# wuxiaolang/Cube_SLAM_wu

Measured on AMD Instinct MI355X. Metric: frames/sec detect_cuboid, higher is better.
Workload: dtype f64

## Files before the change

cube_slam_wu_amd/csrc/detect_kernels.hip:

```cpp
#include <hip/hip_runtime.h>
#include "cs_hip_util.h"

#include <cstdio>
#include <cstdlib>
#include <cstring>

#include "../../include/cubeslam_hip.h"
#include "detect_types.h"

namespace cs {

__device__ __forceinline__ int wave_uniform_i32(int x) { return __builtin_amdgcn_readfirstlane(x); }
__device__ __forceinline__ long long wave_uniform_i64(long long x) {
  const unsigned lo = (unsigned)__builtin_amdgcn_readfirstlane((int)(unsigned)(x & 0xffffffffll)), hi = (unsigned)__builtin_amdgcn_readfirstlane((int)(x >> 32));
  return (long long)(((unsigned long long)hi << 32) | lo);
}
template <typename T>
__device__ __forceinline__ int find_job_wave(const T* __restrict__ prefix, int n, T elem) {
  const T first = sizeof(T) == 8 ? (T)wave_uniform_i64((long long)elem) : (T)wave_uniform_i32((int)elem);
  int lo = 0, hi = n;
  while (hi - lo > 1) {
    const int mid = (lo + hi) >> 1;
    if (prefix[mid] <= first) lo = mid; else hi = mid;
  }
  while (lo + 1 < n && prefix[lo + 1] <= elem) lo++;
  return lo;
}

__device__ __forceinline__ long long xcd_virtual_block() {
  long long nb = gridDim.x, b = blockIdx.x;
  return (b & 7) * (nb >> 3) + (b >> 3);
}

__device__ __attribute__((noinline)) double vp_exact_raw(double dy, double dx) { return cs_atan2(dy, dx); }

__device__ __forceinline__ double vp_exact_unwrapped(const double* __restrict__ mx, const double* __restrict__ my, int i, int ib, double vpxk, double vpyk) {
  const double raw = vp_exact_raw(my[i] - vpyk, mx[i] - vpxk);
  if (i == ib) return raw;
  const double base = vp_exact_raw(my[ib] - vpyk, mx[ib] - vpxk);
  if ((raw - base) < -CS_PI) return raw + 2 * CS_PI;
  if ((raw - base) > CS_PI) return raw - 2 * CS_PI;
  return raw;
}
__device__ __attribute__((noinline)) float vp_rare_unwrapped_f(const double* mx, const double* my, int i, int ib, double vpxk, double vpyk) {
  return (float)vp_exact_unwrapped(mx, my, i, ib, vpxk, vpyk);
}
__device__ __attribute__((noinline)) bool vp_rare_greater(const double* mx, const double* my, int i, int i_ref, int ib, double vpxk, double vpyk) {
  return vp_exact_unwrapped(mx, my, i, ib, vpxk, vpyk) > vp_exact_unwrapped(mx, my, i_ref, ib, vpxk, vpyk);
}
__device__ __attribute__((noinline)) bool vp_rare_less(const double* mx, const double* my, int i, int i_ref, int ib, double vpxk, double vpyk) {
  return vp_exact_unwrapped(mx, my, i, ib, vpxk, vpyk) < vp_exact_unwrapped(mx, my, i_ref, ib, vpxk, vpyk);
}
struct VpExactInlier { float at; int inl; };
__device__ __attribute__((noinline)) VpExactInlier vp_rare_inlier(double dyd, double dxd, double lai, double thre) {
  const double raw = cs_atan2(dyd, dxd);
  const double nrm = normalize_to_pi(raw);
  double d = dabs(lai - nrm);
  d = dmin(d, CS_PI - d);
  return VpExactInlier{(float)raw, d < thre ? 1 : 0};
}

struct VpRun {
  bool have;
  int ib, i_hi, i_lo;
  float base_f, hi_f, lo_f;
  double hx, hy, lx, ly;
};

__device__ __forceinline__ float atan2_float(float fy, float fx, bool* usable) {
  const float PI_F = 3.14159274f, HPI_F = 1.57079637f;
  const float ay = fabsf(fy), ax = fabsf(fx);
  const float hi = fmaxf(ax, ay), lo = fminf(ax, ay);
  const float q = lo * __builtin_amdgcn_rcpf(hi), q2 = q * q;
  float at = -0.01172120f;
  at = __builtin_fmaf(at, q2, 0.05265332f);
  at = __builtin_fmaf(at, q2, -0.11643287f);
  at = __builtin_fmaf(at, q2, 0.19354346f);
  at = __builtin_fmaf(at, q2, -0.33262347f);
  at = __builtin_fmaf(at, q2, 0.99997726f);
  at = at * q;
  if (ay > ax) at = HPI_F - at;
  if (fx < 0.0f) at = PI_F - at;
  if (fy < 0.0f) at = -at;
  *usable = hi > 0.0f && hi < 3.0e38f;
  return at;
}

__device__ __forceinline__ void vp_step(const double* __restrict__ mx, const double* __restrict__ my, int i, double mxi, double myi, double lai,
                                        double vpxk, double vpyk, double thre, float thre_f, VpRun& R) {
  const float PI_F = 3.14159274f, HPI_F = 1.57079637f, M_IN = 1.0e-5f, M_ORD = 2.0e-5f;
  const double dyd = myi - vpyk, dxd = mxi - vpxk;
  bool usable;
  float at = atan2_float((float)dyd, (float)dxd, &usable);
  float nr = at;
  if (at > HPI_F) nr = at - PI_F; else if (at < -HPI_F) nr = at + PI_F;
  float df = fabsf((float)lai - nr);
  df = fminf(df, PI_F - df);
  bool inl = usable && df < thre_f - M_IN;
  if (!(inl || (usable && df > thre_f + M_IN))) { const VpExactInlier x = vp_rare_inlier(dyd, dxd, lai, thre); inl = x.inl != 0; at = x.at; }
  if (inl) {
    if (!R.have) {
      R.have = true; R.ib = i; R.i_hi = i; R.i_lo = i; R.base_f = at; R.hi_f = at; R.lo_f = at; R.hx = dxd; R.hy = dyd; R.lx = dxd; R.ly = dyd;
    } else {
      const float d = at - R.base_f;
      float sh = d < -PI_F ? at + 2.0f * PI_F : d > PI_F ? at - 2.0f * PI_F : at;
      if (fabsf(fabsf(d) - PI_F) < M_ORD) sh = vp_rare_unwrapped_f(mx, my, i, R.ib, vpxk, vpyk);
      if (sh > R.hi_f + M_ORD) { R.hi_f = sh; R.i_hi = i; R.hx = dxd; R.hy = dyd; }
      else if (sh > R.hi_f - M_ORD) {
        const double c = R.hx * dyd - R.hy * dxd, lim = 1.0e-12 * ((dabs(dxd) + dabs(dyd)) * (dabs(R.hx) + dabs(R.hy)));
        const bool greater = c > lim ? true : c < -lim ? false : vp_rare_greater(mx, my, i, R.i_hi, R.ib, vpxk, vpyk);
        if (greater) { R.hi_f = sh; R.i_hi = i; R.hx = dxd; R.hy = dyd; }
      }
      if (sh < R.lo_f - M_ORD) { R.lo_f = sh; R.i_lo = i; R.lx = dxd; R.ly = dyd; }
      else if (sh < R.lo_f + M_ORD) {
        const double c = R.lx * dyd - R.ly * dxd, lim = 1.0e-12 * ((dabs(dxd) + dabs(dyd)) * (dabs(R.lx) + dabs(R.ly)));
        const bool less = c < -lim ? true : c > lim ? false : vp_rare_less(mx, my, i, R.i_lo, R.ib, vpxk, vpyk);
        if (less) { R.lo_f = sh; R.i_lo = i; R.lx = dxd; R.ly = dyd; }
      }
    }
  }
}

struct VpChunk {
  double2 xy[64];
  double ang[64];
  float2 dir[64];
};

template <int K, bool UNIFORM>
__device__ __forceinline__ void vp_support_multi(const double* __restrict__ mx, const double* __restrict__ my, const double* __restrict__ la, int m, VpChunk* ch,
                                                 const double* vpx, const double* vpy, const double* thre, const bool* swapped, bool lane_on, double* out) {
  VpRun R[K];
  float thre_f[K], tan_f[K];
#pragma unroll
  for (int k = 0; k < K; k++) {
    R[k] = VpRun{false, 0, 0, 0, 0.f, 0.f, 0.f, 0., 0., 0., 0.}; thre_f[k] = (float)thre[k];
    tan_f[k] = thre_f[k] < 1.5f ? tanf(thre_f[k] + 1.0e-4f) : __builtin_huge_valf();
  }
  if (UNIFORM) {
    const int lane = threadIdx.x & 63;
    for (int c0 = 0; c0 < m; c0 += 64) {
      const int n = min(64, m - c0);
      __builtin_amdgcn_fence(__ATOMIC_ACQ_REL, "wavefront");
      if (lane < n) {
        const double a = la[c0 + lane];
        ch->xy[lane] = make_double2(mx[c0 + lane], my[c0 + lane]);
        ch->ang[lane] = a;
        ch->dir[lane] = make_float2(cosf((float)a), sinf((float)a));
      }
      __builtin_amdgcn_fence(__ATOMIC_ACQ_REL, "wavefront");
      __builtin_amdgcn_wave_barrier();
      unsigned long long mask[K];
#pragma unroll
      for (int k = 0; k < K; k++) mask[k] = 0;
#pragma unroll 4
      for (int u = 0; u < n; u++) {
        const double2 P = ch->xy[u];
        const float2 ud = ch->dir[u];
#pragma unroll
        for (int k = 0; k < K; k++) {
          const float fx = (float)(P.x - vpx[k]), fy = (float)(P.y - vpy[k]);
          const float cr = fabsf(__builtin_fmaf(fx, ud.y, -(fy * ud.x))), dt = fabsf(__builtin_fmaf(fx, ud.x, fy * ud.y));
          const bool out_for_sure = cr > __builtin_fmaf(tan_f[k], dt, 2.0e-6f * (fabsf(fx) + fabsf(fy)));
          mask[k] |= (unsigned long long)(out_for_sure ? 0 : 1) << u;
        }
      }
#pragma unroll
      for (int k = 0; k < K; k++) {
        unsigned long long mk = lane_on ? mask[k] : 0ull;
        while (__any(mk != 0)) {
          if (mk != 0) {
            const int u = __ffsll((long long)mk) - 1;
            mk &= mk - 1;
            const double2 P = ch->xy[u];
            vp_step(mx, my, c0 + u, P.x, P.y, ch->ang[u], vpx[k], vpy[k], thre[k], thre_f[k], R[k]);
          }
        }
      }
    }
  } else {
    const int mm = lane_on ? m : 0;
    for (int i = 0; i < mm; i++) {
      const double X = mx[i], Y = my[i], A = la[i];
#pragma unroll
      for (int k = 0; k < K; k++) vp_step(mx, my, i, X, Y, A, vpx[k], vpy[k], thre[k], thre_f[k], R[k]);
    }
  }
  const double NaN = __builtin_nan("");
#pragma unroll
  for (int k = 0; k < K; k++) {
    const double ang_hi = R[k].have ? la[R[k].i_hi] : NaN, ang_lo = R[k].have ? la[R[k].i_lo] : NaN;
    out[2 * k] = swapped[k] ? ang_lo : ang_hi;
    out[2 * k + 1] = swapped[k] ? ang_hi : ang_lo;
  }
}

enum { VP3_RPCAP = 32 };

template <int MODE, bool UNIFORM>
__device__ __forceinline__ void vp_support_body(const DetectDeviceView& v, const SweepParams& sp, const JobDesc& jd, int j, long long e, bool on, VpChunk* ch) {
  int rp = 0, y = 0;
  if (on) {
    int local = (int)e - jd.vp_off;
    on = local < jd.RP * jd.Y;
    rp = local / jd.Y; y = local - rp * jd.Y;
  }
  double vpx[3] = {0, 0, 0}, vpy[3] = {0, 0, 0};
  if (on) {
    const RpPose* pose = v.rp + jd.rp_off + rp;
    double cy = v.yaw_cos[jd.yaw_off + y], sy = v.yaw_sin[jd.yaw_off + y];
    const double* A = pose->KinvR;
    double d[3][3] = {{cy, sy, 0.0}, {-sy, cy, 0.0}, {0.0, 0.0, 1.0}};
#pragma unroll
    for (int k = 0; k < 3; k++) {
      double h0 = (A[0] * d[k][0] + A[1] * d[k][1]) + A[2] * d[k][2];
      double h1 = (A[3] * d[k][0] + A[4] * d[k][1]) + A[5] * d[k][2];
      double h2 = (A[6] * d[k][0] + A[7] * d[k][1]) + A[8] * d[k][2];
      vpx[k] = h0 / h2;
      vpy[k] = h1 / h2;
    }
    if (MODE == 0) {
      double* vout = v.vp + 6 * e;
      vout[0] = vpx[0]; vout[1] = vpy[0]; vout[2] = vpx[1]; vout[3] = vpy[1]; vout[4] = vpx[2]; vout[5] = vpy[2];
    }
  }
  const double* mx = v.mid_x + jd.line_off;
  const double* my = v.mid_y + jd.line_off;
  const double* la = v.line_angle + jd.line_off;
  double b6[6];
  const double thre[3] = {sp.vp12_thre_rad, sp.vp12_thre_rad, sp.vp3_thre_rad};
  const bool swapped[3] = {false, true, true};
  vp_support_multi<(MODE == 0 ? 3 : 2), UNIFORM>(mx, my, la, jd.m, ch, vpx, vpy, thre, swapped, on, b6);
  if (!on) return;
  if (MODE == 1) { const double* t3 = v.bound3 + 2 * ((size_t)j * VP3_RPCAP + rp); b6[4] = t3[0]; b6[5] = t3[1]; }
  double* bout = v.bound + 6 * e;
#pragma unroll
  for (int q = 0; q < 6; q++) bout[q] = b6[q];
}

template <int MODE>
__global__ __launch_bounds__(256) void vp_support_kernel(DetectDeviceView v, SweepParams sp, int vp_total) {
  long long e = xcd_virtual_block() * blockDim.x + threadIdx.x;
  const bool on = e < vp_total;
  const int j = find_job_wave<int>(v.vp_prefix, v.n_jobs, on ? (int)e : vp_total - 1);
  const int ju = wave_uniform_i32(j);
  __shared__ VpChunk chunk[4];
  if (__all(j == ju)) vp_support_body<MODE, true>(v, sp, v.jobs[ju], ju, e, on, &chunk[threadIdx.x >> 6]);
  else vp_support_body<MODE, false>(v, sp, v.jobs[j], j, e, on, nullptr);
}

__global__ __launch_bounds__(64) void vp3_support_kernel(DetectDeviceView v, SweepParams sp, int rp_stride) {
  const long long e = (long long)blockIdx.x * 64 + threadIdx.x;
  const int j = (int)(e / rp_stride), rp = (int)(e % rp_stride);
  bool on = j < v.n_jobs;
  JobDesc jd{};
  if (on) { jd = v.jobs[j]; on = rp < jd.RP && jd.Y > 0; }
  double vx = 0, vy = 0;
  if (on) {
    const double* A = (v.rp + jd.rp_off + rp)->KinvR;
    double h0 = (A[0] * 0.0 + A[1] * 0.0) + A[2] * 1.0;
    double h1 = (A[3] * 0.0 + A[4] * 0.0) + A[5] * 1.0;
    double h2 = (A[6] * 0.0 + A[7] * 0.0) + A[8] * 1.0;
    vx = h0 / h2; vy = h1 / h2;
  }
  double o2[2];
  const bool swapped3 = true;
  vp_support_multi<1, false>(v.mid_x + jd.line_off, v.mid_y + jd.line_off, v.line_angle + jd.line_off, on ? jd.m : 0, nullptr, &vx, &vy, &sp.vp3_thre_rad, &swapped3, on, o2);
  if (on) { double* t3 = v.bound3 + 2 * ((size_t)j * VP3_RPCAP + rp); t3[0] = o2[0]; t3[1] = o2[1]; }
}

__global__ __launch_bounds__(256) void vp_points_kernel(DetectDeviceView v, int vp_total) {
  long long e = (long long)blockIdx.x * blockDim.x + threadIdx.x;
  int j = find_job_wave<int>(v.vp_prefix, v.n_jobs, e < vp_total ? (int)e : vp_total - 1);
  if (e >= vp_total) return;
  const JobDesc jd = v.jobs[j];
  int local = (int)e - jd.vp_off;
  if (local >= jd.RP * jd.Y) return;
  int rp = local / jd.Y, y = local - rp * jd.Y;
  const RpPose* pose = v.rp + jd.rp_off + rp;
  double cy = v.yaw_cos[jd.yaw_off + y], sy = v.yaw_sin[jd.yaw_off + y];
  const double* A = pose->KinvR;
  double d[3][3] = {{cy, sy, 0.0}, {-sy, cy, 0.0}, {0.0, 0.0, 1.0}};
  double* vout = v.vp + 6 * e;
#pragma unroll
  for (int k = 0; k < 3; k++) {
    double h0 = (A[0] * d[k][0] + A[1] * d[k][1]) + A[2] * d[k][2];
    double h1 = (A[3] * d[k][0] + A[4] * d[k][1]) + A[5] * d[k][2];
    double h2 = (A[6] * d[k][0] + A[7] * d[k][1]) + A[8] * d[k][2];
    vout[2 * k] = h0 / h2;
    vout[2 * k + 1] = h1 / h2;
  }
}

__device__ __forceinline__ int candidate_one(const DetectDeviceView& v, const SweepParams& sp, const JobDesc& jd, long long tid) {
  const unsigned k = (unsigned)(tid - jd.slot_off);
  const unsigned half = (unsigned)jd.RP * (unsigned)jd.Y * (unsigned)jd.T;
  if (k >= 2 * half) { v.flag[tid] = 0; return 0; }
  const int cfg = (k >= half) ? 2 : 1;
  const unsigned rest = (k >= half) ? k - half : k;
  const unsigned ryu = rest / (unsigned)jd.T;
  const int t = (int)(rest - ryu * (unsigned)jd.T);
  const long long slot = jd.slot_off + (long long)rest * 2 + (cfg - 1);
  const bool enabled = (cfg == 1) ? (sp.consider_config_1 != 0) : (sp.consider_config_2 != 0);
  int flag = 0;
  if (enabled) {
    const double* vp = v.vp + 6 * (long long)(jd.vp_off + (int)ryu);
    V2 c[8];
    flag = build_corners(jd.g, v2(vp[0], vp[1]), v2(vp[2], vp[3]), v2(vp[4], vp[5]), (double)v.top_x[jd.top_off + t], cfg, sp.short_sq_bound, c);
  }
  v.flag[slot] = flag;
  return flag;
}

__global__ __launch_bounds__(256) void candidate_kernel(DetectDeviceView v, SweepParams sp, long long slot_total) {
  long long tid = xcd_virtual_block() * blockDim.x + threadIdx.x;
  bool active = tid < slot_total;
  int flag = 0;
  int j = find_job_wave<long long>(v.slot_prefix, v.n_jobs, active ? tid : slot_total - 1);
  const int ju = wave_uniform_i32(j);
  if (__all(j == ju)) {
    if (active) flag = candidate_one(v, sp, v.jobs[ju], tid);
  } else {
    if (active) flag = candidate_one(v, sp, v.jobs[j], tid);
  }
  unsigned long long valid = __ballot(flag != 0);
  if (valid) {
    int lane = threadIdx.x & 63;
    int j0 = __shfl(j, __ffsll((long long)valid) - 1);
    unsigned long long same = __ballot(flag != 0 && j == j0);
    if (same == valid) {
      if (lane == __ffsll((long long)valid) - 1) atomicAdd(&v.job_valid[j0], __popcll(valid));
    } else if (flag != 0) {
      atomicAdd(&v.job_valid[j], 1);
    }
  }
}

enum { COMPACT_PER = 16 };
enum { CC_TRIP = 4096 };
__global__ __launch_bounds__(256) void candidate_compact_kernel(DetectDeviceView v, SweepParams sp) {
  const int j = blockIdx.x;
  if (j >= v.n_jobs) return;
  __shared__ unsigned char s_flag[CC_TRIP];
  __shared__ int wsum[4];
  const JobDesc& jd = v.jobs[j];
  const int tid = threadIdx.x, lane = tid & 63, wid = tid >> 6;
  const int n_vp = jd.RP * jd.Y;
  for (int e = tid; e < n_vp; e += 256) {
    const int rp = e / jd.Y, y = e - rp * jd.Y;
    const RpPose* pose = v.rp + jd.rp_off + rp;
    const double cy = v.yaw_cos[jd.yaw_off + y], sy = v.yaw_sin[jd.yaw_off + y];
    const double* A = pose->KinvR;
    const double d[3][3] = {{cy, sy, 0.0}, {-sy, cy, 0.0}, {0.0, 0.0, 1.0}};
    double* vout = v.vp + 6 * (long long)(jd.vp_off + e);
#pragma unroll
    for (int k = 0; k < 3; k++) {
      const double h0 = (A[0] * d[k][0] + A[1] * d[k][1]) + A[2] * d[k][2];
      const double h1 = (A[3] * d[k][0] + A[4] * d[k][1]) + A[5] * d[k][2];
      const double h2 = (A[6] * d[k][0] + A[7] * d[k][1]) + A[8] * d[k][2];
      vout[2 * k] = h0 / h2;
      vout[2 * k + 1] = h1 / h2;
    }
  }
  __syncthreads();
  const unsigned half = (unsigned)n_vp * (unsigned)jd.T;
  const unsigned Tu = (unsigned)jd.T;
  const bool fast_div = Tu > 1 && (unsigned long long)half * Tu < (1ull << 32);
  const unsigned inv_T = fast_div ? 0xffffffffu / Tu + 1u : 0u;
  const long long base = v.slot_prefix[j];
  long long run = base;
  const unsigned long long below = (1ull << lane) - 1ull;
  const bool en1 = sp.consider_config_1 != 0, en2 = sp.consider_config_2 != 0;
  for (unsigned r0 = 0; r0 < half; r0 += CC_TRIP / 2) {
#pragma unroll 1
    for (int q = 0; q < 16; q++) {
      const int cfg = 1 + (q >> 3);
      const unsigned rl = (unsigned)(q & 7) * 256u + (unsigned)tid, rest = r0 + rl;
      int flag = 0;
      if (rest < half && (cfg == 1 ? en1 : en2)) {
        const unsigned ryu = fast_div ? __umulhi(rest, inv_T) : rest / Tu;
        const int t = (int)(rest - ryu * Tu);
        const double* vp = v.vp + 6 * (long long)(jd.vp_off + (int)ryu);
        V2 c[8];
        flag = build_corners(jd.g, v2(vp[0], vp[1]), v2(vp[2], vp[3]), v2(vp[4], vp[5]), (double)v.top_x[jd.top_off + t], cfg, sp.short_sq_bound, c);
      }
      s_flag[2 * rl + (unsigned)(cfg - 1)] = (unsigned char)flag;
    }
    __syncthreads();
    int f[COMPACT_PER];
    int wcount = 0;
#pragma unroll
    for (int q = 0; q < COMPACT_PER; q++) {
      f[q] = s_flag[wid * (64 * COMPACT_PER) + q * 64 + lane];
      wcount += __popcll(__ballot(f[q] != 0));
    }
    if (lane == 0) wsum[wid] = wcount;
    __syncthreads();
    int woff = 0, total = 0;
#pragma unroll
    for (int w = 0; w < 4; w++) { const int x = wsum[w]; if (w < wid) woff += x; total += x; }
    long long pos0 = run + woff;
    const long long sl0 = base + 2ll * r0 + wid * (64 * COMPACT_PER) + lane;
#pragma unroll
    for (int q = 0; q < COMPACT_PER; q++) {
      const unsigned long long bal = __ballot(f[q] != 0);
      if (f[q] != 0) {
        const long long pos = pos0 + __popcll(bal & below);
        v.c_slot[pos] = sl0 + q * 64;
        v.c_flag[pos] = f[q] | (j << CAND_JOB_SHIFT);
      }
      pos0 += __popcll(bal);
    }
    run += total;
    __syncthreads();
  }
  const int n_valid = (int)(run - base);
  if (tid == 0) { v.job_valid[j] = n_valid; v.job_cbase[j] = base; }
  const int nblk = (n_valid + 255) >> 8;
  if (nblk > 0) {
    __shared__ int s_at;
    if (tid == 0) s_at = atomicAdd(&v.blk_info[0], nblk);
    __syncthreads();
    const int at = s_at, b0 = (int)(base >> 8);
    for (int k = tid; k < nblk; k += 256) {
      const int left = n_valid - 256 * k;
      v.blk_info[2 + 2 * (long long)(at + k)] = b0 + k;
      v.blk_info[3 + 2 * (long long)(at + k)] = left > 256 ? 256 : left;
    }
  }
}

__device__ __forceinline__ int slot_corners(const DetectDeviceView& v, const JobDesc& jd, long long slot, double short_sq_bound, V2 c[8]) {
  const unsigned local = (unsigned)(slot - jd.slot_off);
  const unsigned rest = local >> 1, ryu = rest / (unsigned)jd.T;
  const int t = (int)(rest - ryu * (unsigned)jd.T);
  const double* vp = v.vp + 6 * (long long)(jd.vp_off + (int)ryu);
  return build_corners(jd.g, v2(vp[0], vp[1]), v2(vp[2], vp[3]), v2(vp[4], vp[5]), (double)v.top_x[jd.top_off + t], (int)(local & 1) + 1, short_sq_bound, c);
}
__device__ __forceinline__ void slot_corners16(const DetectDeviceView& v, long long slot, double short_sq_bound, double out16[16]) {
  int lo = 0, hi = v.n_jobs;
  while (hi - lo > 1) { const int mid = (lo + hi) >> 1; if (v.slot_prefix[mid] <= slot) lo = mid; else hi = mid; }
  V2 c[8];
#pragma unroll
  for (int q = 0; q < 8; q++) c[q] = v2(0.0, 0.0);
  slot_corners(v, v.jobs[lo], slot, short_sq_bound, c);
#pragma unroll
  for (int q = 0; q < 8; q++) { out16[q] = c[q].x; out16[8 + q] = c[q].y; }
}

__device__ __forceinline__ int sel(int cfg, int a, int b) { return cfg ? b : a; }

enum { SCORE_JOBS = 4, SCORE_SUB = 128, SCORE_BINS = SCORE_JOBS * SCORE_SUB };
__device__ __forceinline__ unsigned score_udiv(unsigned n, unsigned d, unsigned inv) { return inv ? __umulhi(n, inv) : n / d; }
template <bool CAP>
__global__ __launch_bounds__(256) void score_kernel(DetectDeviceView v, long long slot_total, double short_sq_bound) {
  __shared__ double C16[16][260];
  double (*CXt)[260] = C16, (*CYt)[260] = C16 + 8;
  const bool cap = CAP;
  long long n_valid = cap ? 256ll * v.blk_info[0] : v.job_cbase[v.n_jobs];
  const long long per_xcd = ((n_valid + 255) / 256 + 7) / 8;
  const long long kx = blockIdx.x >> 3;
  if (kx >= per_xcd) return;
  long long base = ((long long)(blockIdx.x & 7) * per_xcd + kx) * blockDim.x;
  if (base >= n_valid) return;
  if (cap) {
    const int* entry = v.blk_info + 2 + 2 * (base >> 8);
    base = 256ll * entry[0];
    n_valid = base + entry[1];
  }
  __shared__ int hist[SCORE_BINS + 1];
  __shared__ int s_src[256], s_job[256], s_flag[256];
  __shared__ long long s_slot[256];
  {
    const int t0 = threadIdx.x;
    for (int b = t0; b <= SCORE_BINS; b += 256) hist[b] = 0;
    __syncthreads();
    const long long i0 = base + t0;
    long long slot0 = 0;
    int j0 = 0;
    int flag0 = 0;
    if (i0 < n_valid) { slot0 = v.c_slot[i0]; flag0 = v.c_flag[i0]; j0 = flag0 >> CAND_JOB_SHIFT; }
    s_slot[t0] = slot0; s_job[t0] = j0; s_flag[t0] = flag0 & CAND_VP_MASK;
    __syncthreads();
    int key = SCORE_BINS;
    if (i0 < n_valid) {
      const int jq = CAP ? __builtin_amdgcn_readfirstlane(s_job[0]) : j0;
      const int T0 = v.jobs[jq].T;
      const unsigned loc = (unsigned)(slot0 - v.jobs[jq].slot_off);
      const int jrel = j0 - s_job[0];
      const unsigned hq = loc >> 1;
      const unsigned qT = CAP ? score_udiv(hq, (unsigned)T0, ((unsigned long long)v.jobs[jq].RP * v.jobs[jq].Y * T0 * T0 < (1ull << 32) && T0 > 1) ? 0xffffffffu / (unsigned)T0 + 1u : 0u) : hq / (unsigned)T0;
      const int sub = (int)(loc & 1) * T0 + (int)(hq - qT * (unsigned)T0);
      key = (jrel < SCORE_JOBS && sub < SCORE_SUB) ? jrel * SCORE_SUB + sub : SCORE_BINS - 1;
    }
    const int rank = atomicAdd(&hist[key], 1);
    __syncthreads();
    if (t0 < 64) {
      constexpr int PER = (SCORE_BINS + 1 + 63) / 64;
      int loc_sum = 0, vals[PER];
#pragma unroll
      for (int q = 0; q < PER; q++) { const int b = t0 * PER + q; vals[q] = b <= SCORE_BINS ? hist[b] : 0; loc_sum += vals[q]; }
      int incl = loc_sum;
#pragma unroll
      for (int o = 1; o < 64; o <<= 1) { const int y = __shfl_up(incl, o); if (t0 >= o) incl += y; }
      int run = incl - loc_sum;
#pragma unroll
      for (int q = 0; q < PER; q++) { const int b = t0 * PER + q; if (b <= SCORE_BINS) hist[b] = run; run += vals[q]; }
    }
    __syncthreads();
    s_src[hist[key] + rank] = t0;
    __syncthreads();
  }
  const int mine = s_src[threadIdx.x];
  const JobDesc& jd = v.jobs[CAP ? __builtin_amdgcn_readfirstlane(s_job[0]) : s_job[mine]];
  const long long i = base + mine;
  if (i >= n_valid) return;
  const long long slot = s_slot[mine];
  const unsigned local = (unsigned)(slot - jd.slot_off);
  const int cfg = (int)(local & 1);
  const unsigned inv_T = (CAP && jd.T > 1 && (unsigned long long)jd.RP * jd.Y * jd.T * jd.T < (1ull << 32)) ? 0xffffffffu / (unsigned)jd.T + 1u : 0u;
  const unsigned inv_Y = (CAP && jd.Y > 1 && (unsigned long long)jd.RP * jd.Y * jd.Y < (1ull << 32)) ? 0xffffffffu / (unsigned)jd.Y + 1u : 0u;
  const int ry = (int)score_udiv(local >> 1, (unsigned)jd.T, inv_T);
  const int rp = (int)score_udiv((unsigned)ry, (unsigned)jd.Y, inv_Y);
  const int tx = threadIdx.x;
  const double ox = (double)jd.g.el, oy = (double)jd.g.et;
  const float* __restrict__ map = v.maps + jd.map_off;
  {
    V2 cb[8];
    const unsigned rest = local >> 1;
    const double* vp = v.vp + 6 * (long long)(jd.vp_off + ry);
    rebuild_accepted_corners(jd.g, v2(vp[0], vp[1]), v2(vp[2], vp[3]), v2(vp[4], vp[5]), (double)v.top_x[jd.top_off + (int)(rest - (unsigned)ry * (unsigned)jd.T)], cfg + 1,
                             s_flag[mine], cb);
#pragma unroll
    for (int q = 0; q < 8; q++) { CXt[q][tx] = cb[q].x; CYt[q][tx] = cb[q].y; }
  }
  double bnd[6];
  {
    const double* bound = v.bound + 6 * (long long)(jd.vp_off + ry);
#pragma unroll
    for (int q = 0; q < 6; q++) bnd[q] = bound[q];
  }
  float sum_dist = 0;
  const unsigned long long EA = cfg ? 0x004213210ull : 0x443213210ull, EB = cfg ? 0x005450321ull : 0x577450321ull;
  const unsigned long long EW = cfg ? 0x004332222ull : 0x222222222ull;
  const int n_edges = cfg ? 7 : 9;
  const int map_w = jd.map_w;
  constexpr int EU = 3;
  const bool wave_has_cfg1 = __any(cfg == 0);
#pragma unroll 1
  for (int e0 = 0; e0 < n_edges; e0 += EU) {
    float dv[EU][11];
#pragma unroll
    for (int u = 0; u < EU; u++) {
      const int e = e0 + u;
      if (u > 0 && e0 == 6 && !wave_has_cfg1) {
#pragma unroll
        for (int s = 0; s < 11; s++) dv[u][s] = 0.0f;
        continue;
      }
      const int a = (int)((EA >> (4 * e)) & 7), b = (int)((EB >> (4 * e)) & 7);
      const double x1 = CXt[a][tx] - ox, y1 = CYt[a][tx] - oy, x2 = CXt[b][tx] - ox, y2 = CYt[b][tx] - oy;
#pragma unroll
      for (int s = 0; s < 11; s++) {
        double sx, sy;
        if (s == 0) { sx = x2; sy = y2; }
        else if (s == 10) { sx = x1; sy = y1; }
        else if (s == 5) { sx = (x1 + x2) * 0.5; sy = (y1 + y2) * 0.5; }
        else { const double w = (double)s / 10.0; sx = w * x1 + (1 - w) * x2; sy = w * y1 + (1 - w) * y2; }
        dv[u][s] = map[(unsigned)(__mul24((int)sy, map_w) + (int)sx)];
      }
    }
#pragma unroll
    for (int u = 0; u < EU; u++) {
      const int e = e0 + u;
      const float wt = 0.5f * (float)(int)((EW >> (4 * e)) & 7);
      const bool on = e < n_edges;
#pragma unroll
      for (int s = 0; s < 11; s++) { const float nx = sum_dist + dv[u][s] * wt; sum_dist = on ? nx : sum_dist; }
    }
  }
  double total = 0;
  const double not_found_penalty = 30.0 / 180.0 * CS_PI * 2;
  const int ID1[3][4] = {{0, 1, 7, 4}, {3, 0, 4, 5}, {3, 7, 1, 5}}, ID2[3][4] = {{0, 1, 2, 3}, {3, 0, 4, 5}, {2, 4, 1, 5}};
#pragma unroll
  for (int k = 0; k < 3; k++) {
    double b0 = bnd[2 * k], b1 = bnd[2 * k + 1];
    bool v0 = !(b0 != b0), v1 = !(b1 != b1);
    if (v0 || v1) {
#pragma unroll
      for (int ee = 0; ee < 2; ee++) {
        int pa = sel(cfg, ID1[k][2 * ee], ID2[k][2 * ee]), pb = sel(cfg, ID1[k][2 * ee + 1], ID2[k][2 * ee + 1]);
        double ang = normalize_to_pi(cs_atan2(CYt[pb][tx] - CYt[pa][tx], CXt[pb][tx] - CXt[pa][tx]));
        double best = 100;
        if (v0) { double t = dabs(ang - b0); t = dmin(t, CS_PI - t); if (t < best) best = t; }
        if (v1) { double t = dabs(ang - b1); t = dmin(t, CS_PI - t); if (t < best) best = t; }
        total = total + best;
      }
    } else {
      total = total + not_found_penalty;
    }
  }
  V2 c[8];
#pragma unroll
  for (int q = 0; q < 8; q++) c[q] = v2(CXt[q][tx], CYt[q][tx]);
  const RpPose* pose = v.rp + jd.rp_off + rp;
  double p3[3], s3[3];
  lift_to_3d(c, pose->R, pose->t, v.invK + 9 * jd.frame, pose->plane, p3, s3);
  int flag = s_flag[mine];
  if (s3[0] < 0 || s3[1] < 0 || s3[2] < 0) flag |= CAND_NEG_SCALE;
  v.c_flag[i] = flag;
  v.c_dist[i] = (double)sum_dist / jd.diag;
  v.c_angle[i] = total;
  v.c_skew[i] = dmax(s3[0], s3[1]) / dmin(s3[0], s3[1]);
}

__global__ __launch_bounds__(1024) void scan_jobs_kernel(const int* job_valid, long long* job_cbase, int n_jobs) {
  __shared__ long long wsum[16];
  __shared__ long long carry_s;
  if (threadIdx.x == 0) carry_s = 0;
  __syncthreads();
  int lane = threadIdx.x & 63, wid = threadIdx.x >> 6;
  for (int base = 0; base < n_jobs; base += 1024) {
    int i = base + threadIdx.x;
    long long x = (i < n_jobs) ? job_valid[i] : 0;
    long long incl = x;
#pragma unroll
    for (int o = 1; o < 64; o <<= 1) {
      long long y = __shfl_up(incl, o);
      if (lane >= o) incl += y;
    }
    if (lane == 63) wsum[wid] = incl;
    __syncthreads();
    long long woff = 0;
    for (int w = 0; w < wid; w++) woff += wsum[w];
    long long carry = carry_s;
    if (i < n_jobs) job_cbase[i] = carry + woff + incl - x;
    __syncthreads();
    if (threadIdx.x == 1023) carry_s = carry + woff + incl;
    __syncthreads();
  }
  if (threadIdx.x == 0) job_cbase[n_jobs] = carry_s;
}

__global__ __launch_bounds__(256) void compact_kernel(DetectDeviceView v) {
  int j = blockIdx.x;
  if (j >= v.n_jobs) return;
  __shared__ int wsum[4];
  const long long s0 = v.slot_prefix[j], s1 = v.slot_prefix[j + 1];
  long long run = v.job_cbase[j];
  const int lane = threadIdx.x & 63, wid = threadIdx.x >> 6;
  const unsigned long long below = (1ull << lane) - 1ull;
  for (long long base = s0; base < s1; base += 256 * COMPACT_PER) {
    const long long w0 = base + (long long)wid * (64 * COMPACT_PER) + lane;
    int f[COMPACT_PER];
    int wcount = 0;
#pragma unroll
    for (int q = 0; q < COMPACT_PER; q++) {
      const long long sl = w0 + q * 64;
      f[q] = (sl < s1) ? v.flag[sl] : 0;
      wcount += __popcll(__ballot(f[q] != 0));
    }
    if (lane == 0) wsum[wid] = wcount;
    __syncthreads();
    int woff = 0, total = 0;
#pragma unroll
    for (int w = 0; w < 4; w++) { const int x = wsum[w]; if (w < wid) woff += x; total += x; }
    long long pos0 = run + woff;
#pragma unroll
    for (int q = 0; q < COMPACT_PER; q++) {
      const unsigned long long bal = __ballot(f[q] != 0);
      if (f[q] != 0) {
        const long long pos = pos0 + __popcll(bal & below);
        v.c_slot[pos] = w0 + q * 64;
        v.c_flag[pos] = f[q] | (j << CAND_JOB_SHIFT);
      }
      pos0 += __popcll(bal);
    }
    run += total;
    __syncthreads();
  }
}

__global__ __launch_bounds__(256) void compact_count_kernel(DetectDeviceView v, int* __restrict__ cnt, int maxc) {
  const int j = blockIdx.x, c = blockIdx.y;
  __shared__ int wsum[4];
  const long long end = v.slot_prefix[j + 1], s0 = v.slot_prefix[j] + (long long)c * (256 * COMPACT_PER), s1 = (s0 + 256 * COMPACT_PER < end) ? s0 + 256 * COMPACT_PER : end;
  int n = 0;
  for (long long sl = s0 + threadIdx.x; sl < s1; sl += 256) n += v.flag[sl] != 0;
#pragma unroll
  for (int o = 32; o > 0; o >>= 1) n += __shfl_down(n, o);
  if ((threadIdx.x & 63) == 0) wsum[threadIdx.x >> 6] = n;
// ... 1298 lines not shown
```

Measured before the change: 536,100.

## Add f32 interval-arithmetic prefilter for corner validity with exact f64 fallback

Adds a float32 evaluation of the cuboid corner-building test that carries error bounds, returning accept, reject, or unsure. Only unsure candidates go through the original double-precision build_corners. In the compact kernel the unsure slots are gathered into a shared-memory list and rechecked in a second pass so the f64 work is not divergent. This aims to replace most of the slow FP64 arithmetic with FP32 work. It adds shared-memory atomics and an extra barrier per tile, and correctness depends on the error bounds being conservative.

```diff
diff --git a/cube_slam_wu_amd/csrc/cs_geom_f32.h b/cube_slam_wu_amd/csrc/cs_geom_f32.h
--- /dev/null
+++ b/cube_slam_wu_amd/csrc/cs_geom_f32.h
@@ -0,0 +1,182 @@
+#pragma once
+#include "cs_geom.h"
+
+namespace cs {
+
+enum { CS_CORNERS_UNSURE = 255 };
+
+#ifdef CS_GEOM_F32_ZERO_MARGIN
+#define CS_F32_U 0.0f
+#define CS_F32_DIVU 0.0f
+#define CS_F32_ETA 0.0f
+#define CS_F32_INFL 1.0f
+#else
+#define CS_F32_U 6.0e-8f
+#define CS_F32_DIVU 3.0e-7f
+#define CS_F32_ETA 1.0e-30f
+#define CS_F32_INFL 1.001f
+#endif
+
+#if defined(__HIP_DEVICE_COMPILE__)
+#define CS_F32_FMA(a, b, c) __builtin_fmaf((a), (b), (c))
+#define CS_F32_RCP(x) __builtin_amdgcn_rcpf(x)
+#else
+#define CS_F32_FMA(a, b, c) ((a) * (b) + (c))
+#define CS_F32_RCP(x) (1.0f / (x))
+#endif
+
+struct FE {
+  float v, e;
+};
+struct P2F {
+  FE x, y;
+};
+
+CS_HD float f32_abs(float a) { return __builtin_fabsf(a); }
+CS_HD FE fe_exact(int i) { return FE{(float)i, 0.0f}; }
+CS_HD FE fe_in(double d) { const float v = (float)d; return FE{v, CS_F32_FMA(CS_F32_U, f32_abs(v), CS_F32_ETA)}; }
+CS_HD FE fe_in_maybe_exact(double d) {
+  const float v = (float)d;
+  const bool exact = (double)v == d && (f32_abs(v) >= 1.0f || v == 0.0f);
+  return FE{v, exact ? 0.0f : CS_F32_FMA(CS_F32_U, f32_abs(v), CS_F32_ETA)};
+}
+CS_HD FE fe_sub(FE a, FE b) { const float v = a.v - b.v; return FE{v, CS_F32_FMA(CS_F32_U, f32_abs(v), a.e + b.e)}; }
+CS_HD FE fe_add(FE a, FE b) { const float v = a.v + b.v; return FE{v, CS_F32_FMA(CS_F32_U, f32_abs(v), a.e + b.e)}; }
+CS_HD FE fe_mul(FE a, FE b) {
+  const float v = a.v * b.v;
+  float e = CS_F32_FMA(CS_F32_U, f32_abs(v), CS_F32_ETA);
+  e = CS_F32_FMA(f32_abs(b.v), a.e, e);
+  e = CS_F32_FMA(f32_abs(a.v) + a.e, b.e, e);
+  return FE{v, e};
+}
+CS_HD FE fe_div(FE a, FE b) {
+  const float ab = f32_abs(b.v);
+  const float v = a.v * CS_F32_RCP(b.v);
+  const float room = ab - b.e;
+  float e = CS_F32_FMA(CS_F32_DIVU, f32_abs(v), CS_F32_ETA);
+  e = CS_F32_FMA(CS_F32_FMA(f32_abs(v), b.e, a.e), CS_F32_RCP(room), e);
+  const bool ok = room > 0.0f && ab < 1.0e30f;
+  return FE{v, ok ? e : __builtin_huge_valf()};
+}
+
+struct Tri {
+  bool yes, no;
+};
+CS_HD Tri tri_and(Tri a, Tri b) { return Tri{a.yes && b.yes, a.no || b.no}; }
+CS_HD Tri fe_less(FE x, FE t) {
+  const float m = CS_F32_INFL * (x.e + t.e);
+  return Tri{t.v - x.v > m, x.v - t.v > m};
+}
+CS_HD Tri fe_within(FE x, float l, float r) {
+  const float m = CS_F32_INFL * x.e;
+  return Tri{x.v - l > m && r - x.v > m, l - x.v > m || x.v - r > m};
+}
+CS_HD Tri fe_nonneg(FE x) {
+  const float m = CS_F32_INFL * x.e;
+  return Tri{x.v > m, -x.v > m};
+}
+
+CS_HD Tri f32_short(P2F a, P2F b, FE bound) {
+  const FE dx = fe_sub(a.x, b.x), dy = fe_sub(a.y, b.y);
+  const float v = CS_F32_FMA(dx.v, dx.v, dy.v * dy.v);
+  const float s = dx.e + dy.e;
+  float p = f32_abs(dy.v) * dy.e;
+  p = CS_F32_FMA(f32_abs(dx.v), dx.e, p);
+  float e = CS_F32_FMA(3.0f * CS_F32_U, v, CS_F32_ETA);
+  e = CS_F32_FMA(s, s, e);
+  e = CS_F32_FMA(2.0f, p, e);
+  return fe_less(FE{v, e}, bound);
+}
+
+CS_HD Tri f32_hit_vertical(P2F s, P2F p, float bx, float y0, float y1, FE* hit_y) {
+  const FE dx = fe_sub(p.x, s.x), dy = fe_sub(p.y, s.y);
+  const FE lam = fe_div(fe_sub(FE{bx, 0.0f}, s.x), dx);
+  const FE ty = fe_add(s.y, fe_mul(lam, dy));
+  *hit_y = ty;
+  return tri_and(fe_nonneg(lam), fe_within(ty, y0, y1));
+}
+CS_HD Tri f32_hit_horizontal(P2F s, P2F p, float by, float x0, float x1, FE* hit_x) {
+  const FE dx = fe_sub(p.x, s.x), dy = fe_sub(p.y, s.y);
+  const FE lam = fe_div(fe_sub(FE{by, 0.0f}, s.y), dy);
+  const FE tx = fe_add(s.x, fe_mul(lam, dx));
+  *hit_x = tx;
+  return tri_and(fe_nonneg(lam), fe_within(tx, x0, x1));
+}
+CS_HD P2F f32_line_intersect(P2F a1, P2F a2, P2F b1, P2F b2) {
+  const FE X2_X1 = fe_sub(a2.x, a1.x), Y2_Y1 = fe_sub(a2.y, a1.y);
+  const FE X4_X3 = fe_sub(b2.x, b1.x), Y4_Y3 = fe_sub(b2.y, b1.y);
+  const FE X1_X3 = fe_sub(a1.x, b1.x), Y1_Y3 = fe_sub(a1.y, b1.y);
+  const FE num = fe_sub(fe_mul(X4_X3, Y1_Y3), fe_mul(Y4_Y3, X1_X3));
+  const FE den = fe_sub(fe_mul(Y4_Y3, X2_X1), fe_mul(X4_X3, Y2_Y1));
+  const FE u_a = fe_div(num, den);
+  return P2F{fe_add(a1.x, fe_mul(X2_X1, u_a)), fe_add(a1.y, fe_mul(Y2_Y1, u_a))};
+}
+CS_HD Tri f32_inside_box(P2F p, int l, int t, int r, int b) { return tri_and(fe_within(p.x, (float)l, (float)r), fe_within(p.y, (float)t, (float)b)); }
+
+CS_HD int corners_predecide(const BoxGeom& g, V2 vp1d, V2 vp2d, V2 vp3d, double top_x, int config_id, double short_sq_bound) {
+  const int LIM = 1 << 24;
+  if (g.top == g.down || g.left == g.right || g.left < 0 || g.top < 0 || g.right < 0 || g.down < 0 || g.right >= LIM || g.down >= LIM || g.left >= LIM || g.top >= LIM ||
+      g.el <= -LIM || g.el >= LIM || g.et <= -LIM || g.et >= LIM || g.er <= -LIM || g.er >= LIM || g.eb <= -LIM || g.eb >= LIM)
+    return CS_CORNERS_UNSURE;
+  const float left = (float)g.left, top = (float)g.top, right = (float)g.right, down = (float)g.down;
+  const P2F vp1{fe_in(vp1d.x), fe_in(vp1d.y)}, vp2{fe_in(vp2d.x), fe_in(vp2d.y)}, vp3{fe_in(vp3d.x), fe_in(vp3d.y)};
+  const FE bound = fe_in(short_sq_bound);
+  const P2F c1{fe_in_maybe_exact(top_x), FE{top, 0.0f}};
+  bool pending = false;
+  bool rejected = false;
+#define CS_F32_REJECT_IF(t) do { const Tri t_ = (t); rejected |= t_.yes; pending |= !t_.no; } while (0)
+#define CS_F32_REJECT_UNLESS(t) do { const Tri t_ = (t); rejected |= t_.no; pending |= !t_.yes; } while (0)
+#define CS_F32_CHECKPOINT() do { if (rejected) return 0; } while (0)
+  FE yR, yL;
+  const Tri hR = f32_hit_vertical(vp1, c1, right, top, down, &yR);
+  const Tri hL = f32_hit_vertical(vp1, c1, left, top, down, &yL);
+  int vp1_pos;
+  if (hR.yes) vp1_pos = 1;
+  else if (hR.no && hL.no) return 0;
+  else if (hR.no && hL.yes) vp1_pos = 2;
+  else return CS_CORNERS_UNSURE;
+  const bool right_first = vp1_pos == 1;
+  const float side1 = right_first ? right : left, side2 = right_first ? left : right;
+  const P2F c2{FE{side1, 0.0f}, right_first ? yR : yL};
+  CS_F32_REJECT_IF(f32_short(c1, c2, bound));
+  CS_F32_CHECKPOINT();
+  const bool k1 = config_id == 1;
+  const P2F P = k1 ? c1 : c2;
+  FE yH;
+  CS_F32_REJECT_UNLESS(f32_hit_vertical(vp2, P, side2, top, down, &yH));
+  const P2F H{FE{side2, 0.0f}, yH};
+  CS_F32_REJECT_IF(f32_short(P, H, bound));
+  const P2F L = k1 ? f32_line_intersect(vp2, c2, vp1, H) : f32_line_intersect(vp1, H, vp2, c1);
+  CS_F32_REJECT_UNLESS(f32_inside_box(L, g.left, k1 ? g.top : g.et, g.right, k1 ? g.down : g.eb));
+  CS_F32_REJECT_IF(f32_short(L, H, bound));
+  CS_F32_REJECT_IF(f32_short(L, k1 ? c2 : c1, bound));
+  CS_F32_CHECKPOINT();
+  const P2F c3 = k1 ? L : H, c4 = k1 ? H : L;
+  FE x5;
+  CS_F32_REJECT_UNLESS(f32_hit_horizontal(vp3, c3, down, left, right, &x5));
+  const P2F c5{x5, FE{down, 0.0f}};
+  CS_F32_REJECT_IF(f32_short(c3, c5, bound));
+  CS_F32_CHECKPOINT();
+  const P2F c6 = f32_line_intersect(vp2, c5, vp3, c2);
+  CS_F32_REJECT_UNLESS(f32_inside_box(c6, g.el, g.et, g.er, g.eb));
+  CS_F32_REJECT_IF(f32_short(c6, c2, bound));
+  CS_F32_REJECT_IF(f32_short(c6, c5, bound));
+  CS_F32_CHECKPOINT();
+  const P2F c7 = f32_line_intersect(vp1, c6, vp3, c1);
+  CS_F32_REJECT_UNLESS(f32_inside_box(c7, g.el, g.et, g.er, g.eb));
+  CS_F32_REJECT_IF(f32_short(c7, c1, bound));
+  CS_F32_REJECT_IF(f32_short(c7, c6, bound));
+  CS_F32_CHECKPOINT();
+  const P2F c8 = f32_line_intersect(vp1, c5, vp2, c7);
+  CS_F32_REJECT_UNLESS(f32_inside_box(c8, g.el, g.et, g.er, g.eb));
+  CS_F32_REJECT_IF(f32_short(c8, c4, bound));
+  CS_F32_REJECT_IF(f32_short(c8, c5, bound));
+  CS_F32_REJECT_IF(f32_short(c8, c7, bound));
+  CS_F32_CHECKPOINT();
+#undef CS_F32_REJECT_IF
+#undef CS_F32_REJECT_UNLESS
+#undef CS_F32_CHECKPOINT
+  return pending ? (int)CS_CORNERS_UNSURE : vp1_pos;
+}
+
+}
diff --git a/cube_slam_wu_amd/csrc/detect_kernels.hip b/cube_slam_wu_amd/csrc/detect_kernels.hip
--- a/cube_slam_wu_amd/csrc/detect_kernels.hip
+++ b/cube_slam_wu_amd/csrc/detect_kernels.hip
@@ -7,6 +7,7 @@
 
 #include "../../include/cubeslam_hip.h"
 #include "detect_types.h"
+#include "cs_geom_f32.h"
 
 namespace cs {
 
@@ -292,6 +293,10 @@
   }
 }
 
+__device__ __attribute__((noinline)) int corners_exact_flag(const BoxGeom* g, const double* __restrict__ vp, double top_x, int cfg, double short_sq_bound) {
+  V2 c[8];
+  return build_corners(*g, v2(vp[0], vp[1]), v2(vp[2], vp[3]), v2(vp[4], vp[5]), top_x, cfg, short_sq_bound, c);
+}
 __device__ __forceinline__ int candidate_one(const DetectDeviceView& v, const SweepParams& sp, const JobDesc& jd, long long tid) {
   const unsigned k = (unsigned)(tid - jd.slot_off);
   const unsigned half = (unsigned)jd.RP * (unsigned)jd.Y * (unsigned)jd.T;
@@ -305,8 +310,13 @@
   int flag = 0;
   if (enabled) {
     const double* vp = v.vp + 6 * (long long)(jd.vp_off + (int)ryu);
-    V2 c[8];
-    flag = build_corners(jd.g, v2(vp[0], vp[1]), v2(vp[2], vp[3]), v2(vp[4], vp[5]), (double)v.top_x[jd.top_off + t], cfg, sp.short_sq_bound, c);
+    const double top_x = (double)v.top_x[jd.top_off + t];
+#ifdef CS_DIAG
+    flag = CS_CORNERS_UNSURE;
+#else
+    flag = corners_predecide(jd.g, v2(vp[0], vp[1]), v2(vp[2], vp[3]), v2(vp[4], vp[5]), top_x, cfg, sp.short_sq_bound);
+#endif
+    if (flag == CS_CORNERS_UNSURE) flag = corners_exact_flag(&jd.g, vp, top_x, cfg, sp.short_sq_bound);
   }
   v.flag[slot] = flag;
   return flag;
@@ -342,6 +352,8 @@
   const int j = blockIdx.x;
   if (j >= v.n_jobs) return;
   __shared__ unsigned char s_flag[CC_TRIP];
+  __shared__ unsigned short s_unsure[CC_TRIP];
+  __shared__ int s_n_unsure;
   __shared__ int wsum[4];
   const JobDesc& jd = v.jobs[j];
   const int tid = threadIdx.x, lane = tid & 63, wid = tid >> 6;
@@ -371,22 +383,49 @@
   long long run = base;
   const unsigned long long below = (1ull << lane) - 1ull;
   const bool en1 = sp.consider_config_1 != 0, en2 = sp.consider_config_2 != 0;
+  if (tid == 0) s_n_unsure = 0;
+  __syncthreads();
   for (unsigned r0 = 0; r0 < half; r0 += CC_TRIP / 2) {
 #pragma unroll 1
     for (int q = 0; q < 16; q++) {
       const int cfg = 1 + (q >> 3);
       const unsigned rl = (unsigned)(q & 7) * 256u + (unsigned)tid, rest = r0 + rl;
+      const unsigned at = 2 * rl + (unsigned)(cfg - 1);
       int flag = 0;
       if (rest < half && (cfg == 1 ? en1 : en2)) {
+#ifdef CS_DIAG
+        flag = CS_CORNERS_UNSURE;
+#else
         const unsigned ryu = fast_div ? __umulhi(rest, inv_T) : rest / Tu;
         const int t = (int)(rest - ryu * Tu);
         const double* vp = v.vp + 6 * (long long)(jd.vp_off + (int)ryu);
-        V2 c[8];
-        flag = build_corners(jd.g, v2(vp[0], vp[1]), v2(vp[2], vp[3]), v2(vp[4], vp[5]), (double)v.top_x[jd.top_off + t], cfg, sp.short_sq_bound, c);
-      }
-      s_flag[2 * rl + (unsigned)(cfg - 1)] = (unsigned char)flag;
-    }
-    __syncthreads();
+        flag = corners_predecide(jd.g, v2(vp[0], vp[1]), v2(vp[2], vp[3]), v2(vp[4], vp[5]), (double)v.top_x[jd.top_off + t], cfg, sp.short_sq_bound);
+#endif
+      }
+      s_flag[at] = (unsigned char)flag;
+      const unsigned long long ub = __ballot(flag == CS_CORNERS_UNSURE);
+      if (ub) {
+        const int first = __ffsll((long long)ub) - 1;
+        int ubase = 0;
+        if (lane == first) ubase = atomicAdd(&s_n_unsure, __popcll(ub));
+        ubase = __shfl(ubase, first);
+        if (flag == CS_CORNERS_UNSURE) s_unsure[ubase + __popcll(ub & below)] = (unsigned short)at;
+      }
+    }
+    __syncthreads();
+    const int n_unsure = s_n_unsure;
+    if (n_unsure > 0) {
+      for (int i = tid; i < n_unsure; i += 256) {
+        const unsigned at = s_unsure[i];
+        const int cfg = 1 + (int)(at & 1u);
+        const unsigned rest = r0 + (at >> 1);
+        const unsigned ryu = fast_div ? __umulhi(rest, inv_T) : rest / Tu;
+        const int t = (int)(rest - ryu * Tu);
+        s_flag[at] = (unsigned char)corners_exact_flag(&jd.g, v.vp + 6 * (long long)(jd.vp_off + (int)ryu), (double)v.top_x[jd.top_off + t], cfg, sp.short_sq_bound);
+      }
+      __syncthreads();
+      if (tid == 0) s_n_unsure = 0;
+    }
     int f[COMPACT_PER];
     int wcount = 0;
 #pragma unroll
```

Result: slower. 471,500 (-12.0%).
